# nv-dvl/nerfmatch

Measured on AMD Instinct MI355X. Metric: rays*samples/sec, higher is better.
Workload: dtype fp16x3 (fp16 MFMA on hi/lo-split fp32 operands, three products per fp32 product, fp32 accumulate; fp32 everywhere else)

## Files before the change

### nerfmatch_amd/csrc/nerf_fwd_bf16.hip

```cpp
#include "nerf_split_chain.h"

namespace {
using namespace nmbf;
using nmsample::HALF_PI_F32, nmsample::SCAN_TILE, nmsample::frustum, nmsample::ray_consts, nmsample::lift_var, nmsample::ipe_fast, nmsample::view_row_value;
using nmsample::alpha_of, nmsample::trans_factor, nmsample::sigmoid, nmsample::scan_before_barrier, nmsample::scan_after_barrier, nmsample::scan_carry;
using nmsample::first_max;
static_assert(TILE == SCAN_TILE, "the compositing scan of nerf_sample.h spans two wavefronts");

template <int PART>
__device__ __forceinline__ void tap_prefetch(Ctx& cx) {
  if constexpr (PART == 0) __builtin_amdgcn_s_barrier();
  const char* src = reinterpret_cast<const char*>(cx.tapw);
#pragma unroll
  for (int q = (PART == 0 ? 0 : 4); q < (PART == 0 ? 4 : 7); ++q) {
    const char* sp = src + q * 4096;
    const float* dp = q < 4 ? cx.tap_ring + q * 1024 : cx.tap_ipe + (q - 4) * 1024;
    const unsigned lds = (unsigned)__builtin_amdgcn_readfirstlane((int)(unsigned)(size_t)(const __attribute__((address_space(3))) float*)dp);
    unsigned m0_saved;
    asm volatile("s_mov_b32 %0, m0\n\ts_mov_b32 m0, %1\n\tglobal_load_lds_dwordx4 %2, off\n\tglobal_load_lds_dwordx4 %2, off offset:1024\n\t"
                 "global_load_lds_dwordx4 %2, off offset:2048\n\tglobal_load_lds_dwordx4 %2, off offset:3072\n\ts_mov_b32 m0, %0"
                 : "=&s"(m0_saved) : "s"(lds), "v"(sp) : "memory");
  }
}

// ... 67 lines not shown
#pragma unroll
    for (int i = 0; i < 8; ++i) s3[8 * b + i] = o[i];
  }
  float lo8[8], hi8[8];
#pragma unroll
  for (int i = 0; i < 8; ++i) { lo8[i] = s3[i]; hi8[i] = s3[8 + i]; }
  quad_add8<2>(lo8); quad_add8<2>(hi8);
  float s4[8];
#pragma unroll
  for (int i = 0; i < 8; ++i) s4[i] = (lane & 2) ? hi8[i] : lo8[i];
  float t8[8] = {s4[0], s4[1], s4[2], s4[3], s4[4], s4[5], s4[6], s4[7]};
  quad_add8<1>(t8);
  return (lane & 1) ? f32x4{t8[4], t8[5], t8[6], t8[7]} : f32x4{t8[0], t8[1], t8[2], t8[3]};
}
__device__ __forceinline__ f32x4 reduce_scatter_32rows(float (&v)[128], int lane) {
  float s1[64];
#pragma unroll
  for (int i = 0; i < 64; ++i) s1[i] = reduce_scatter_step16(v[i], v[64 + i]);
  return reduce_scatter_16pairs(s1, lane);
}

#define NM_MLP_DONE_WAIT() __builtin_amdgcn_s_waitcnt(0x0070)
#define NM_EPI_BARRIER() asm volatile("s_waitcnt lgkmcnt(0)\n\ts_barrier" ::: "memory")
template <int P>
__device__ __forceinline__ void nerf_fwd_body(const NerfArgs& a) {
  __shared__ __attribute__((aligned(16))) float sm[LDS_TOTAL];
  float* const sm_small = sm + LDS_SMALL;
  float* const ring = sm + LDS_RING;
  float* const sm_ipe = sm + LDS_IPE;
  float* const sm_sigma = sm + LDS_SCR;
  float* const sm_rgb = sm_sigma + TILE;
  float* const sm_t0 = sm_rgb + 3 * TILE;
  float* const sm_t1 = sm_t0 + TILE;
  float* const sm_mean = sm_t1 + TILE;
  float* const sm_dn = sm_mean + 3 * TILE;
  float* const sm_w = sm_dn + TILE;
  float* const sm_misc = sm_w + TILE;
  float* const sm_part = sm_misc + 32;
  float* const sm_feat = sm + LDS_FEAT;
  float* const sm_ex = sm + LDS_EX;
  int* const sm_lray = reinterpret_cast<int*>(sm + LDS_LEFT);
  float* const sm_lT = sm + LDS_LEFT + TILE;
  unsigned* const sm_rng = reinterpret_cast<unsigned*>(sm + LDS_RNG);

  const int tid = threadIdx.x, lane = tid & 63, wave = tid >> 6, s = lane & 31, hi = lane >> 5;
  const bool tail_ok = a.left && !(a.tail_viol && *a.tail_viol != 0);
  const int S = a.S, R = a.R;
  const int Sa = tail_ok ? a.Sa : S;
// ... 68 lines not shown
      sm_dn[js] = dnorm;
    }

    ring_open<P>(blob_slots, ring, wave, lane);

    {
      const float ipe_scale = sm_small[OFF_INSCALE];
      const float phl = hi ? HALF_PI_F32 : 0.f;
      park_ipe<P>(sm_ipe + wave * (XS * 2 * 64 * 4) + lane * 4, [&](int idx) {
        const int ax = idx % 3;
        const float sc = (float)(1 << (idx / 3));
        float v = ipe_fast(mean[ax] * sc + phl, var[ax], sc);
        if constexpr (P == 2) v *= ipe_scale;
        return v;
      });
    }

    TRACE(2);
    Ctx cx;
    cx.blob_slots = blob_slots; cx.ring = ring; cx.sm_small = sm_small;
    cx.tapw = reinterpret_cast<f32x4*>(a.ws) + ((size_t)blockIdx.x * 4 + wave) * 32 * 64 + lane;
    cx.nslots = nslots; cx.wave = wave; cx.lane = lane; cx.hi = hi; cx.tap = need_tap ? tap : -1; cx.g = 0; cx.sig_part = 0.f;
    cx.vmax = 0.f; cx.rng = sm_rng + tid; cx.sc = 1.f;
    const bool early = need_rgb && !lo_pass && tap == 7 && a.feat && !a.sfeat;
    cx.tap_pref = need_tap && !lo_pass && !early; cx.rgb = need_rgb;
    cx.tap_ring = ring + wave * SLOT_FLOATS; cx.tap_ipe = sm_ipe + wave * (XS * 2 * 64 * 4);
    if constexpr (is_split<P>()) {
      ring_open_wait<P>(cx);
    } else {
      ring_acquire<P>(blob_slots, 0, nslots, ring, wave, lane);
    }
    load_half<P>(cx.opA, ring, lane, 0);
    if constexpr (P == 1) load_half<1>(cx.opB, ring, lane, 1);
    const float* ipe_src = sm_ipe + wave * (XS * 2 * 64 * 4) + lane * 4;

    auto composite_weights = [&]() __attribute__((always_inline)) {
      const int tid2 = launder(threadIdx.x), lane2 = tid2 & 63, wave2 = tid2 >> 6;
      float alpha = 0.f, incl = 1.f;
      if (tid2 < TILE) {
        alpha = alpha_of(sm_sigma[tid2], (sm_t1[tid2] - sm_t0[tid2]) * sm_dn[tid2]);
        incl = scan_before_barrier(trans_factor(alpha), lane2, wave2, SP, sm_misc);
      }
      NM_EPI_BARRIER();
      if (tid2 < TILE) {
        const float excl = scan_after_barrier(incl, lane2, wave2, SP, sm_misc, carryT);
        sm_w[tid2] = alpha * excl;
        const int r2 = tid2 / SP, ray2 = bid * nr + r2;
// ... 62 lines not shown
#pragma unroll
      for (int cq = 0; cq < HS; ++cq) {
        const f32x4 b0 = *reinterpret_cast<const f32x4*>(bl + (cq >> 2) * 32 + 8 * (cq & 3));
        const f32x4 b1 = *reinterpret_cast<const f32x4*>(bl + (4 + (cq >> 2)) * 32 + 8 * (cq & 3));
#pragma unroll
        for (int e = 0; e < 4; ++e) {
          const float x = mult * __builtin_fmaxf(__builtin_fmaf(c.hv[4 * cq + e], s7, b0[e]), 0.f);
          const float y = mult * __builtin_fmaxf(__builtin_fmaf(c.hv[64 + 4 * cq + e], s7, b1[e]), 0.f);
          s1[4 * cq + e] = reduce_scatter_step16(x, y);
        }
      }
      const f32x4 sum4 = reduce_scatter_16pairs(s1, jl);
      const int r = jl & 31;
      float* prow = sm_feat + (jl >> 5) * 256 + 4 * hl;
      *reinterpret_cast<f32x4*>(prow + (r >> 2) * 32 + 16 * ((r >> 1) & 1) + 8 * (r & 1)) = sum4;
    };
    const Tap7InRegisters<decltype(tap7_early)> tap7{early, tap7_early};
    f32x16 acc[8];
    ipe_steps<P, true>(acc, cx, ipe_src);
    finish_layer<P>(acc, 0, cx);
    TRACE(3);
#pragma unroll 1
    for (int l = 1; l < 8; ++l) {
      layer_pass<P>(acc, l, cx, ipe_src, tap7);
      TRACE(3 + l);
    }
    float c_r = 0.f, c_g = 0.f, c_b = 0.f;
    if (!need_rgb) {
      if (cx.tap == 7) dump_tap(7, cx);
      NM_MLP_DONE_WAIT();
      if (cx.tap_pref) tap_prefetch<0>(cx);
      alpha_head(cx);
      if (cx.tap_pref) tap_prefetch<1>(cx);
    } else {
      const int hh = launder(lane) >> 5;
      const float* exr = sm_ex + launder(rl) * 48 + 8 * hh;
      f32x16 av[4];
      views_hidden<P>(av, cx);
      fold_range<P>(cx, 7);
      bf16x8 exh[VS], exl[VS];
#pragma unroll
      for (int e = 0; e < VS; ++e) {
        float v8[8];
        if (!lo_pass) {
          const f32x4 e0 = *reinterpret_cast<const f32x4*>(exr + 16 * e), e1 = *reinterpret_cast<const f32x4*>(exr + 16 * e + 4);
          v8[0] = e0[0]; v8[1] = e0[1]; v8[2] = e0[2]; v8[3] = e0[3]; v8[4] = e1[0]; v8[5] = e1[1]; v8[6] = e1[2]; v8[7] = e1[3];
        } else {
          const float* rq = a.rays + (size_t)launder(rc) * 12 + 8;
          const float vd0 = rq[0], vd1 = rq[1], vd2 = rq[2];
#pragma unroll
          for (int i = 0; i < 8; ++i) {
            const int f = 16 * e + 8 * hh + i;
            const int ax = f % 3;
            float v = view_row_value(f, ax == 0 ? vd0 : ax == 1 ? vd1 : vd2, a.app_row);
            if constexpr (P == 2) v *= sm_small[OFF_INSCALE + (f < 27 ? 1 : 2)];
            v8[i] = v;
          }
        }
        if constexpr (is_split<P>()) split8_p<P>(v8, exh[e], exl[e]);
        else exh[e] = exl[e] = pack8_f16(v8);
      }
// ... 188 lines not shown
      if (q == 0) { if (a.acc) a.acc[ray2] = red_acc; }
      else if (q <= 3) { if (a.rgb && need_rgb) a.rgb[(size_t)ray2 * 3 + (q - 1)] = a.white_bg ? red_acc + (1.0f - accv) : red_acc; }
      else if (q == 4) { if (a.depth) a.depth[ray2] = red_acc; }
      else { if (a.pts) a.pts[(size_t)ray2 * 3 + (q - 5)] = red_acc; }
    }
  }
  TRACE(17);
  if (left) nleft += (R - bid * nr) < nr ? (R - bid * nr) : nr;
  bid += gridDim.x;
  }
  if constexpr (P == 2) {
    __syncthreads();
    if (a.status && tid < NRANGE) {
      unsigned m = 0u;
      for (int i = 0; i < 256; ++i) m = max(m, sm_rng[tid * 256 + ((i + 32 * tid) & 255)]);
      if (m) atomicMax(reinterpret_cast<unsigned*>(a.status) + 1 + tid, m);
      if (m >= __float_as_uint(F16_MAX)) atomicOr(a.status, 1);
    }
  }
}

__global__ void __launch_bounds__(256, 1) nerf_fwd_bf16x3_kernel(NerfArgs a) { nerf_fwd_body<0>(a); }
__global__ void __launch_bounds__(256, 1) nerf_fwd_fp16x1_kernel(NerfArgs a) { nerf_fwd_body<1>(a); }
__global__ void __launch_bounds__(256, 1) nerf_fwd_fp16x3_kernel(NerfArgs a) { nerf_fwd_body<2>(a); }

}

extern "C" size_t nm_nerf_workspace_bytes_bf16x3(void) { return (size_t)WS_WORKGROUPS * TILE * 256 * sizeof(float); }

static int nerf_fwd_split(int mode, const void* blob, const float* rays, const float* t, const float* app_row, int R, int S, int tap_layer,
                          int white_bg, float var_scale, int flags, float* weights, float* feat, float* pts, float* rgb, float* depth,
                          float* acc, float* raw, float* sample_feat, void* workspace, const int* zero_tail_violation, nmStream_t stream,
                          int* status = nullptr) {
  NM_CHECK_ARG(blob && rays && t && weights && R > 0 && S > 0);
  if (!(S == 32 || S == 64 || (S % 128) == 0)) return NM_ERR_UNSUPPORTED;
  if (tap_layer > 7) return NM_ERR_ARG;
  if ((feat || sample_feat) && !workspace) return NM_ERR_WORKSPACE;
  NerfArgs a;
  a.ws = (float*)workspace;
  a.blob = (const char*)blob; a.rays = rays; a.t = t; a.app_row = app_row;
  a.weights = weights; a.feat = feat; a.pts = pts; a.rgb = rgb; a.depth = depth; a.acc = acc; a.raw = raw; a.sfeat = sample_feat;
  a.R = R; a.S = S; a.tap = tap_layer; a.white_bg = white_bg; a.flags = flags; a.var_scale = var_scale;
  a.status = status;
  const bool zero_tail = (flags & NM_NERF_ZERO_TAIL) && (S == 64 || S == 128 || (S >= 256 && S % 256 == 0)) && !raw && !sample_feat &&
                         !(flags & NM_NERF_FEAT_MAX);
  a.Sa = zero_tail ? S / 2 : S;
  a.left = zero_tail ? 1 : 0;
  const int SP = a.Sa < TILE ? a.Sa : TILE, nr = TILE / SP;
  a.ntiles = (R + nr - 1) / nr;
  const int SPf = S < TILE ? S : TILE, nrf = TILE / SPf;
  a.ntiles_full = (R + nrf - 1) / nrf;
  a.tail_viol = zero_tail ? zero_tail_violation : nullptr;
  const int ncu = nm_stream_cus(stream);
  const int grid = a.ntiles < ncu ? a.ntiles : (ncu < WS_WORKGROUPS ? ncu : WS_WORKGROUPS);
  if (mode == 1) nerf_fwd_fp16x1_kernel<<<grid, 256, 0, (hipStream_t)stream>>>(a);
  else if (mode == 2) nerf_fwd_fp16x3_kernel<<<grid, 256, 0, (hipStream_t)stream>>>(a);
  else nerf_fwd_bf16x3_kernel<<<grid, 256, 0, (hipStream_t)stream>>>(a);
  return nm_launch_status();
}

extern "C" int nm_nerf_fwd_bf16x3(const void* blob, const float* rays, const float* t, const float* app_row, int R, int S,
                                  int tap_layer, int white_bg, float var_scale, int flags, float* weights, float* feat, float* pts,
                                  float* rgb, float* depth, float* acc, float* raw, float* sample_feat, void* workspace,
                                  const int* zero_tail_violation, nmStream_t stream) {
  return nerf_fwd_split(0, blob, rays, t, app_row, R, S, tap_layer, white_bg, var_scale, flags, weights, feat, pts, rgb, depth, acc, raw,
                        sample_feat, workspace, zero_tail_violation, stream);
}

extern "C" int nm_nerf_fwd_fp16x1(const void* blob, const float* rays, const float* t, const float* app_row, int R, int S,
                                  int tap_layer, int white_bg, float var_scale, int flags, float* weights, float* feat, float* pts,
                                  float* rgb, float* depth, float* acc, float* raw, float* sample_feat, void* workspace,
                                  const int* zero_tail_violation, nmStream_t stream) {
  return nerf_fwd_split(1, blob, rays, t, app_row, R, S, tap_layer, white_bg, var_scale, flags, weights, feat, pts, rgb, depth, acc, raw,
                        sample_feat, workspace, zero_tail_violation, stream);
}

extern "C" int nm_nerf_fwd_fp16x3(const void* blob, const float* rays, const float* t, const float* app_row, int R, int S,
                                  int tap_layer, int white_bg, float var_scale, int flags, float* weights, float* feat, float* pts,
                                  float* rgb, float* depth, float* acc, float* raw, float* sample_feat, void* workspace,
// ... 5 lines not shown
```

### nerfmatch_amd/csrc/nerf_split_chain.h

```cpp
#pragma once
#include "nerf_bf16_common.h"

namespace nmbf {

template <int P> constexpr bool is_bf16() { return P == 0 || P == 4; }
template <int P> constexpr bool has_gates() { return P == 4; }
typedef _Float16 f16x8 __attribute__((ext_vector_type(8)));
typedef _Float16 f16x2 __attribute__((ext_vector_type(2)));
template <int P>
__device__ __forceinline__ f32x16 mfma_p(const bf16x8& a, const bf16x8& b, const f32x16& c) {
  if constexpr (is_bf16<P>()) return MFMA_BF16(a, b, c);
  else return __builtin_amdgcn_mfma_f32_32x32x16_f16(__builtin_bit_cast(f16x8, a), __builtin_bit_cast(f16x8, b), c, 0, 0, 0);
}
template <int P> constexpr bool is_split() { return P != 1; }
template <int P> constexpr int slot_bytes() { return is_split<P>() ? SLOT_BYTES : SLOT_BYTES / 2; }
template <int P> constexpr int slot_floats() { return slot_bytes<P>() / 4; }
template <int P> constexpr int ring_slots() { return is_split<P>() ? NRING : 2 * NRING; }
template <int P> constexpr int ring_ahead() { return is_split<P>() ? 4 : 6; }
constexpr float F16_MAX = 65504.0f;
__device__ __forceinline__ void split8_f16(const float (&v)[8], bf16x8& hi, bf16x8& lo) {
  f16x8 h8, l8;
#pragma unroll
  for (int i = 0; i < 8; ++i) {
    const float c = __builtin_amdgcn_fmed3f(v[i], -F16_MAX, F16_MAX);
// ... 49 lines not shown
  auto* dst = (__attribute__((address_space(3))) void*)(ring_slot<P>(ring, g) + wave * (slot_floats<P>() / 4));
  __builtin_amdgcn_global_load_lds(src, dst, 16, 0, 0);
  __builtin_amdgcn_global_load_lds(src, dst, 16, 1024, 0);
  if constexpr (is_split<P>()) {
    __builtin_amdgcn_global_load_lds(src, dst, 16, 2048, 0);
    __builtin_amdgcn_global_load_lds(src, dst, 16, 3072, 0);
  }
}

template <int P>
__device__ __forceinline__ void ring_acquire(const char* blob_slots, int g, int nslots, float* ring, int wave, int lane) {
  if constexpr (is_split<P>()) {
    NM_WAIT_VMCNT(4);
  } else {
    NM_WAIT_VMCNT(10);
  }
  __builtin_amdgcn_s_barrier();
  if constexpr (is_split<P>()) dma_slot<P>(blob_slots, g + ring_ahead<P>(), ring, wave, lane);
}

__device__ __forceinline__ void ring_acquire_two() {
  asm volatile("s_waitcnt vmcnt(0) lgkmcnt(0)" ::: "memory");
  __builtin_amdgcn_s_barrier();
}

__device__ __forceinline__ void ring_acquire_pair(const char* blob_slots, int g, float* ring, int wave, int lane) {
  NM_WAIT_VMCNT(6);
  __builtin_amdgcn_s_barrier();
  dma_slot<1>(blob_slots, g + 6, ring, wave, lane);
  dma_slot<1>(blob_slots, g + 7, ring, wave, lane);
}

struct OpHalf {
  bf16x8 h[4], l[4];
};

template <int P>
__device__ __forceinline__ void load_half(OpHalf& d, const float* slot, int lane, int p) {
  const u32x4* s4 = reinterpret_cast<const u32x4*>(slot) + lane;
#pragma unroll
  for (int o = 0; o < 4; ++o) {
    if constexpr (is_split<P>()) {
      d.h[o] = __builtin_bit_cast(bf16x8, s4[((4 * p + o) * 2 + 0) * 64]);
      d.l[o] = __builtin_bit_cast(bf16x8, s4[((4 * p + o) * 2 + 1) * 64]);
    } else {
      d.h[o] = __builtin_bit_cast(bf16x8, s4[(4 * p + o) * 64]);
    }
  }
}

struct Ctx {
  const char* blob_slots;
  float* ring;
  const float* sm_small;
  f32x4* tapw;
  bool tap_pref;
  bool rgb;
  float* tap_ring;
  float* tap_ipe;
  int nslots, wave, lane, hi;
  int tap;
  int g;
  unsigned dma_voff;
  unsigned dma_lds;
  OpHalf opA;
  OpHalf opB;
  f32x4 hb0, hb1;
  Unit xn;
  float sig_part;
  float sc;
  float vmax;
  unsigned* rng;
  u32x4* gptr;
  unsigned gbits[4];
  float hv[128];
};

template <int P>
__device__ __forceinline__ void ring_request(const Ctx& cx, int g, int j) {
  const int slot = g + 2 + (j >> 2);
  const char* base = cx.blob_slots + (size_t)slot * slot_bytes<P>();
  const unsigned lds = cx.dma_lds + (unsigned)(slot & (ring_slots<P>() - 1)) * slot_bytes<P>();
  unsigned m0_saved;
#define NM_DMA_PIECE(OFS)                                                                                                        \
  asm volatile("s_mov_b32 %0, m0\n\ts_mov_b32 m0, %1\n\tglobal_load_lds_dwordx4 %2, %3 offset:" #OFS "\n\ts_mov_b32 m0, %0" \
               : "=&s"(m0_saved) : "s"(lds), "v"(cx.dma_voff), "s"(base) : "memory")
  switch (j & 3) {
    case 0: NM_DMA_PIECE(0); break;
    case 1: NM_DMA_PIECE(1024); break;
    case 2: NM_DMA_PIECE(2048); break;
    default: NM_DMA_PIECE(3072); break;
  }
#undef NM_DMA_PIECE
}
template <int P>
__device__ __forceinline__ void ring_open(const char* blob_slots, float* ring, int wave, int lane) {
#pragma unroll
  for (int g0 = 0; g0 < (is_split<P>() ? 2 : ring_ahead<P>()); ++g0) dma_slot<P>(blob_slots, g0, ring, wave, lane);
}
template <int P>
__device__ __forceinline__ void ring_open_wait(Ctx& cx) {
  cx.dma_voff = (unsigned)(cx.wave * (slot_bytes<P>() / 4) + cx.lane * 16);
  const float* q = cx.ring + cx.wave * (slot_floats<P>() / 4);
  cx.dma_lds = (unsigned)__builtin_amdgcn_readfirstlane((int)(unsigned)(size_t)(const __attribute__((address_space(3))) float*)q);
  NM_WAIT_VMCNT(0);
  __builtin_amdgcn_s_barrier();
}

__device__ __forceinline__ unsigned gate_byte(const u32x4& h) {
  const unsigned w0 = h[0], w1 = h[1], w2 = h[2], w3 = h[3];
  unsigned m0, m1, m2, m3;
  const unsigned one = 0x00010001u;
  asm("v_pk_min_u16 %0, %1, %2" : "=v"(m0) : "v"(w0), "v"(one));
  asm("v_pk_min_u16 %0, %1, %2" : "=v"(m1) : "v"(w1), "v"(one));
  asm("v_pk_min_u16 %0, %1, %2" : "=v"(m2) : "v"(w2), "v"(one));
  asm("v_pk_min_u16 %0, %1, %2" : "=v"(m3) : "v"(w3), "v"(one));
  const unsigned t = m0 | (m1 << 1) | (m2 << 2) | (m3 << 3);
  return (t & 0xfu) | ((t >> 12) & 0xf0u);
}

template <bool BF, class W> __device__ __forceinline__ void unit_seq(W& w, int c);
template <bool EVEN, bool BF, class W> __device__ __forceinline__ void unit_step8(W& w, int t);
template <int P>
struct UnitWork {
  Ctx& cx;
  Unit& out;
  int u, lo_;
  float floor_v;
  f32x4 b0, b1;
  float sc;
  float v8[8];
  float f0, f1;
  float r0[4], r1[4];
  __device__ __forceinline__ void bias() {
    const int ob = u >> 1, m = u & 1;
    const float* bl = cx.sm_small + OFF_BIAS + lo_ * 256 + ob * 32 + 16 * m + 4 * cx.hi;
    b0 = *reinterpret_cast<const f32x4*>(bl); b1 = *reinterpret_cast<const f32x4*>(bl + 8);
  }
  __device__ __forceinline__ float act(int e, float b) const {
    const float h = cx.hv[(u >> 1) * 16 + 8 * (u & 1) + e];
    if constexpr (is_bf16<P>()) return __builtin_fmaxf(h + b, floor_v);
    else if constexpr (P == 1) return __builtin_amdgcn_fmed3f(h + b, floor_v, F16_MAX);
    else return __builtin_amdgcn_fmed3f(__builtin_fmaf(h, sc, b), floor_v, F16_MAX);
  }
  __device__ __forceinline__ void range(int j) {
    if constexpr (P == 2) asm("v_max3_f32 %0, |%1|, |%2|, %0" : "+v"(cx.vmax) : "v"(v8[j]), "v"(v8[4 + j]));
  }
  __device__ __forceinline__ void ra(int j) { v8[j] = act(j, b0[j]); pin(v8[j]); }
  __device__ __forceinline__ void rb(int j) { v8[4 + j] = act(4 + j, b1[j]); range(j); pin(v8[4 + j]); }
  __device__ __forceinline__ void relu(int j) {
    v8[j] = act(j, b0[j]); v8[4 + j] = act(4 + j, b1[j]);
    range(j);
    pin(v8[j]); pin(v8[4 + j]);
  }
  __device__ __forceinline__ void hi(int p) {
    unsigned hp;
    if constexpr (is_bf16<P>()) {
      hp = pack_bf16(v8[2 * p], v8[2 * p + 1]);
      f0 = __uint_as_float(hp << 16);
      f1 = __uint_as_float(hp & 0xffff0000u);
// ... 4 lines not shown
    if constexpr (is_bf16<P>()) { pin(f0); pin(f1); }
    out.h[p] = hp;
  }
  __device__ __forceinline__ void rem(int p) {
    if constexpr (is_bf16<P>()) {
      r0[p] = v8[2 * p] - f0; r1[p] = v8[2 * p + 1] - f1;
      pin(r0[p]); pin(r1[p]);
    } else {
      asm volatile("v_fma_mix_f32 %0, %1, -1.0, %2 op_sel:[0,0,0] op_sel_hi:[1,0,0]" : "=v"(r0[p]) : "v"(out.h[p]), "v"(v8[2 * p]));
      asm volatile("v_fma_mix_f32 %0, %1, -1.0, %2 op_sel:[1,0,0] op_sel_hi:[1,0,0]" : "=v"(r1[p]) : "v"(out.h[p]), "v"(v8[2 * p + 1]));
    }
  }
  __device__ __forceinline__ void lo(int p) {
    unsigned lp = is_bf16<P>() ? pack_bf16(r0[p], r1[p]) : pack_f16(r0[p], r1[p]);
    pin(lp);
    out.l[p] = lp;
  }
  __device__ __forceinline__ void gates() {
    if constexpr (has_gates<P>()) {
      const unsigned t = gate_byte(out.h);
      cx.gbits[u >> 2] |= t << (8 * (u & 3));
    }
  }
  __device__ __forceinline__ void seq(int c) { unit_seq<is_bf16<P>()>(*this, c); }
  template <bool EVEN> __device__ __forceinline__ void step8(int t) { unit_step8<EVEN, is_bf16<P>()>(*this, t); }
  __device__ __forceinline__ void prefetch() { bias(); }
  __device__ __forceinline__ void operator()(int j) {
    if (j < 4) relu(j);
    else if constexpr (P == 1) {
      if (j < 8) {
        unsigned hp = pack_f16(v8[2 * (j - 4)], v8[2 * (j - 4) + 1]);
        pin(hp);
        out.h[j - 4] = hp;
      }
    } else if (!(j & 1)) hi((j - 4) >> 1);
    else {
      rem((j - 5) >> 1); lo((j - 5) >> 1);
      if (j == 11) gates();
    }
  }
};
template <bool BF, class W>
__device__ __forceinline__ void unit_seq(W& w, int c) {
  switch (c) {
    case 0: w.bias(); break;
    case 2: w.ra(0); break;
    case 3: w.rb(0); break;
    case 4: w.ra(1); break;
// ... 25 lines not shown
      case 18: if constexpr (BF) { w.rem(2); } break;
      case 19: if constexpr (BF) { w.hi(3); w.lo(2); } break;
      case 20: if constexpr (BF) { w.rem(3); } break;
      case 21: if constexpr (BF) { w.lo(3); } break;
      case 22: if constexpr (BF) { w.gates(); } break;
      default: break;
    }
  }
}
template <int P>
__device__ __forceinline__ void fold_range(Ctx& cx, int slot) {
  if constexpr (P == 2) {
    const unsigned addr = (unsigned)(size_t)(const __attribute__((address_space(3))) unsigned*)(cx.rng + slot * 256);
    asm volatile("ds_max_u32 %0, %1" :: "v"(addr), "v"(__float_as_uint(cx.vmax)) : "memory");
    cx.vmax = 0.f;
  }
}
struct NoWork {
  __device__ __forceinline__ void prefetch() {}
  __device__ __forceinline__ void operator()(int) {}
  __device__ __forceinline__ void seq(int) {}
  template <bool EVEN> __device__ __forceinline__ void step8(int) {}
};
constexpr int take_n(int s) { return s == 0 ? 4 : s == 1 ? 2 : s <= 4 ? 3 : s == 10 ? 2 : 5; }
constexpr int take_before(int s) {
  int n = 0;
  for (int k = 0; k < s; ++k) n += take_n(k);
  return n;
}
constexpr int TAKE_HIDDEN = take_before(12);
__device__ __forceinline__ const float* unit0_bias(const Ctx& cx, int l) { return cx.sm_small + OFF_BIAS + l * 256 + 4 * cx.hi; }
template <int P>
struct AccTake {
  const f32x16 (&acc)[8];
  Ctx& cx;
  int l;
  __device__ __forceinline__ void prefetch() {}
  __device__ __forceinline__ void operator()(int j) {
#pragma unroll
    for (int k = 0; k < 8; ++k) {
      const int i = 8 * j + k;
      if (i < 64) cx.hv[i] = acc_read(acc[i >> 4][i & 15]);
    }
  }
  __device__ __forceinline__ void seq(int) {}
  template <bool EVEN> __device__ __forceinline__ void step8(int t) {
    if (t < 12) return;
    const int s = t - 12;
#pragma unroll
    for (int k = 0; k < take_n(s); ++k) {
      const int i = take_before(s) + k;
      cx.hv[i] = acc_read(acc[i >> 4][i & 15]);
    }
    if (s == 10) {
      const float* bl = unit0_bias(cx, l);
      cx.hb0 = *reinterpret_cast<const f32x4*>(bl); cx.hb1 = *reinterpret_cast<const f32x4*>(bl + 8);
    }
  }
};
template <int P>
__device__ __forceinline__ UnitWork<P> unit_work(int u, int lo, Ctx& cx, Unit& out) {
  return UnitWork<P>{cx, out, u, lo, lo < 8 ? 0.f : (!is_bf16<P>() ? -F16_MAX : -__builtin_inff()), {}, {}, cx.sc, {}, 0.f, 0.f, {}, {}};
}

template <int P>
__device__ __forceinline__ void finish_layer(const f32x16 (&acc)[8], int l, Ctx& cx) {
  if constexpr (is_split<P>()) {
#pragma unroll
    for (int i = TAKE_HIDDEN; i < 64; ++i) cx.hv[i] = acc_read(acc[i >> 4][i & 15]);
  }
#pragma unroll
  for (int ob = 4; ob < 8; ++ob)
#pragma unroll
    for (int r = 0; r < 16; ++r) cx.hv[ob * 16 + r] = acc_read(acc[ob][r]);
  if constexpr (P == 2)
    cx.sc = __builtin_bit_cast(float, __builtin_amdgcn_readfirstlane(__builtin_bit_cast(int, cx.sm_small[OFF_SCALE + l])));
  UnitWork<P> w = unit_work<P>(0, l, cx, cx.xn);
  if constexpr (is_split<P>()) {
    w.b0 = cx.hb0; w.b1 = cx.hb1;
#pragma unroll
    for (int j = 0; j < 4; ++j) w.relu(j);
#pragma unroll
    for (int p = 0; p < 4; ++p) {
      w.hi(p);
      if constexpr (is_bf16<P>()) w.rem(p);
    }
    if constexpr (!is_bf16<P>()) {
#pragma unroll
      for (int p = 0; p < 4; ++p) w.rem(p);
    }
#pragma unroll
    for (int p = 0; p < 4; ++p) w.lo(p);
    w.gates();
  } else {
    w.prefetch();
#pragma unroll
    for (int j = 0; j < 12; ++j) w(j);
  }
}

__device__ __forceinline__ void alpha_head(Ctx& cx) {
  const float* bl = cx.sm_small + OFF_BIAS + 7 * 256 + 4 * cx.hi;
  const float* wa = cx.sm_small + OFF_WALPHA + 4 * cx.hi;
  const float s7 = cx.sm_small[OFF_SCALE + 7];
  float p0 = 0.f, p1 = 0.f, p2 = 0.f, p3 = 0.f;
#pragma unroll
  for (int ob = 0; ob < 8; ++ob)
#pragma unroll
    for (int q = 0; q < 4; ++q) {
      const f32x4 b = *reinterpret_cast<const f32x4*>(bl + ob * 32 + 8 * q);
      const f32x4 w4v = *reinterpret_cast<const f32x4*>(wa + ob * 32 + 8 * q);
      p0 = NM_FMA(__builtin_fmaxf(__builtin_fmaf(cx.hv[ob * 16 + 4 * q + 0], s7, b[0]), 0.f), w4v[0], p0);
      p1 = NM_FMA(__builtin_fmaxf(__builtin_fmaf(cx.hv[ob * 16 + 4 * q + 1], s7, b[1]), 0.f), w4v[1], p1);
      p2 = NM_FMA(__builtin_fmaxf(__builtin_fmaf(cx.hv[ob * 16 + 4 * q + 2], s7, b[2]), 0.f), w4v[2], p2);
      p3 = NM_FMA(__builtin_fmaxf(__builtin_fmaf(cx.hv[ob * 16 + 4 * q + 3], s7, b[3]), 0.f), w4v[3], p3);
    }
  cx.sig_part = (p0 + p1) + (p2 + p3);
}

__device__ __forceinline__ void dump_tap(int lo, Ctx& cx) {
  const float* bl = cx.sm_small + OFF_BIAS + lo * 256 + 4 * cx.hi;
  const float sl = cx.sm_small[OFF_SCALE + lo];
  auto* tp = (__attribute__((address_space(1))) f32x4*)cx.tapw;
#pragma unroll
  for (int ob = 0; ob < 8; ++ob) {
    f32x4 v[4];
#pragma unroll
    for (int q = 0; q < 4; ++q) {
      const f32x4 b = *reinterpret_cast<const f32x4*>(bl + ob * 32 + 8 * q);
#pragma unroll
      for (int e = 0; e < 4; ++e) v[q][e] = __builtin_fmaxf(__builtin_fmaf(cx.hv[ob * 16 + 4 * q + e], sl, b[e]), 0.f);
    }
#pragma unroll
    for (int q = 0; q < 4; ++q) tp[q * 64] = v[q];
    tp += 256;
    pin(tp);
  }
}

__device__ __forceinline__ bf16x8 load_op1(const float* slot, int lane, int blk) {
  return __builtin_bit_cast(bf16x8, (reinterpret_cast<const u32x4*>(slot) + lane)[blk * 64]);
// ... 19 lines not shown
  acc[5] = mfma_p<1>(B.h[1], x, FIRST ? zero : acc[5]); NM_SB;
  work(0); work(1); NM_SB;
  acc[6] = mfma_p<1>(B.h[2], x, FIRST ? zero : acc[6]); NM_SB;
  work(2); work(3); work(4); NM_SB;
  acc[7] = mfma_p<1>(B.h[3], x, FIRST ? zero : acc[7]); NM_SB;
  work(5); work(6); work(7); NM_SB;
  cx.g = g + 1;
}

template <int P>
__device__ __forceinline__ void load_pair(OpHalf& d, const float* slot, int lane, int p, int o) {
  const u32x4* s4 = reinterpret_cast<const u32x4*>(slot) + lane;
  d.h[o] = __builtin_bit_cast(bf16x8, s4[((4 * p + o) * 2 + 0) * 64]);
  d.l[o] = __builtin_bit_cast(bf16x8, s4[((4 * p + o) * 2 + 1) * 64]);
}
template <int P, bool FIRST>
__device__ __forceinline__ f32x16 mfma_k(int k, const OpHalf& a, const bf16x8& xh, const bf16x8& xl, const f32x16& c) {
  const f32x16 zero = {0.f, 0.f, 0.f, 0.f, 0.f, 0.f, 0.f, 0.f, 0.f, 0.f, 0.f, 0.f, 0.f, 0.f, 0.f, 0.f};
  if (k < 4) return mfma_p<P>(a.h[k], xh, FIRST ? zero : c);
  if (k < 8) return mfma_p<P>(a.h[k & 3], xl, c);
  return mfma_p<P>(a.l[k & 3], xh, c);
}

template <int P, bool FIRST, bool EVEN, class Work>
__device__ __forceinline__ void slot_step8(f32x16 (&acc)[8], Ctx& cx, const bf16x8& xh, const bf16x8& xl, Work work) {
  if constexpr (P == 1) {
    slot_step8_one<FIRST, EVEN>(acc, cx, xh, work);
    return;
  }
  const int g = cx.g;
  const OpHalf A = cx.opA;
  OpHalf B;
  const float* cur = cx.ring + (g & (NRING - 1)) * SLOT_FLOATS;
  const float* nxt = cx.ring + ((g + 1) & (NRING - 1)) * SLOT_FLOATS;
#pragma unroll
  for (int k = 0; k < 12; ++k) {
    acc[k & 3] = mfma_k<P, FIRST>(k, A, xh, xl, acc[k & 3]);
    __builtin_amdgcn_sched_barrier(0);
    if (k < 4) load_pair<P>(B, cur, cx.lane, 1, k);
    if constexpr (EVEN) {
      if (k >= 4) ring_request<P>(cx, g, k - 4);
    }
    work.template step8<EVEN>(k);
    __builtin_amdgcn_sched_barrier(0);
  }
  if constexpr (!EVEN) {
    ring_acquire_two();
    __builtin_amdgcn_sched_barrier(0);
  }
#pragma unroll
  for (int k = 0; k < 12; ++k) {
    acc[4 + (k & 3)] = mfma_k<P, FIRST>(k, B, xh, xl, acc[4 + (k & 3)]);
    __builtin_amdgcn_sched_barrier(0);
    if (k >= 1 && k <= 4) load_pair<P>(cx.opA, nxt, cx.lane, 0, k - 1);
    work.template step8<EVEN>(12 + k);
    __builtin_amdgcn_sched_barrier(0);
  }
  cx.g = g + 1;
}

template <bool FIRST, bool ACQ, class Work>
__device__ __forceinline__ void slot_step4_one(f32x16 (&acc)[4], Ctx& cx, const bf16x8& x, Work work) {
  const f32x16 zero = {0.f, 0.f, 0.f, 0.f, 0.f, 0.f, 0.f, 0.f, 0.f, 0.f, 0.f, 0.f, 0.f, 0.f, 0.f, 0.f};
  const int g = cx.g;
  const OpHalf C = cx.opA;
  const float* nxt = ring_slot<1>(cx.ring, g + 1);
  acc[0] = mfma_p<1>(C.h[0], x, FIRST ? zero : acc[0]); NM_SB;
  if constexpr (ACQ) ring_acquire_pair(cx.blob_slots, g, cx.ring, cx.wave, cx.lane);
  NM_SB;
  acc[1] = mfma_p<1>(C.h[1], x, FIRST ? zero : acc[1]); NM_SB;
#pragma unroll
  for (int o = 0; o < 4; ++o) cx.opA.h[o] = load_op1(nxt, cx.lane, o);
  work.prefetch(); NM_SB;
  acc[2] = mfma_p<1>(C.h[2], x, FIRST ? zero : acc[2]); NM_SB;
  work(0); work(1); work(2); work(3); NM_SB;
  acc[3] = mfma_p<1>(C.h[3], x, FIRST ? zero : acc[3]); NM_SB;
  work(4); work(5); work(6); work(7); NM_SB;
// ... 19 lines not shown
      if (k >= 4) ring_request<P>(cx, g, k - 4);
    }
    work.seq(k);
    __builtin_amdgcn_sched_barrier(0);
  }
  cx.g = g + 1;
}

template <int P, bool FIRST, bool EVEN, class W0, class W1>
__device__ __forceinline__ void slot_step4x2(f32x16 (&av)[4], Ctx& cx, const bf16x8& x0h, const bf16x8& x0l, Unit& u1, W0 w0, W1 w1) {
  const int g = cx.g;
  const OpHalf A = cx.opA;
  OpHalf B;
  const float* cur = cx.ring + (g & (NRING - 1)) * SLOT_FLOATS;
  const float* nxt = cx.ring + ((g + 1) & (NRING - 1)) * SLOT_FLOATS;
#pragma unroll
  for (int k = 0; k < 12; ++k) {
    av[k & 3] = mfma_k<P, FIRST>(k, A, x0h, x0l, av[k & 3]);
    __builtin_amdgcn_sched_barrier(0);
    if (k >= 1 && k <= 4) load_pair<P>(B, cur, cx.lane, 1, k - 1);
    if constexpr (EVEN) {
      if (k >= 4) ring_request<P>(cx, g, k - 4);
    }
    w0.seq(k);
    __builtin_amdgcn_sched_barrier(0);
  }
  if constexpr (!EVEN) {
    ring_acquire_two();
    __builtin_amdgcn_sched_barrier(0);
  }
  const bf16x8 x1h = __builtin_bit_cast(bf16x8, u1.h), x1l = __builtin_bit_cast(bf16x8, u1.l);
#pragma unroll
  for (int k = 0; k < 12; ++k) {
    av[k & 3] = mfma_k<P, false>(k, B, x1h, x1l, av[k & 3]);
    __builtin_amdgcn_sched_barrier(0);
    if (k >= 1 && k <= 4) load_pair<P>(cx.opA, nxt, cx.lane, 0, k - 1);
    w1.seq(k);
    __builtin_amdgcn_sched_barrier(0);
  }
  cx.g = g + 1;
}

template <int P>
__device__ __forceinline__ void views_hidden(f32x16 (&av)[4], Ctx& cx) {
  if constexpr (is_split<P>()) {
#pragma unroll
    for (int sl = 0; sl < HS / 2; ++sl) {
      const Unit x0 = cx.xn;
      Unit u1;
      const bf16x8 x0h = __builtin_bit_cast(bf16x8, x0.h), x0l = __builtin_bit_cast(bf16x8, x0.l);
      if (sl == 0) slot_step4x2<P, true, true>(av, cx, x0h, x0l, u1, unit_work<P>(1, 7, cx, u1), unit_work<P>(2, 7, cx, cx.xn));
      else if (sl + 1 == HS / 2) slot_step4x2<P, false, false>(av, cx, x0h, x0l, u1, unit_work<P>(2 * sl + 1, 7, cx, u1), NoWork{});
      else if (sl & 1) slot_step4x2<P, false, false>(av, cx, x0h, x0l, u1, unit_work<P>(2 * sl + 1, 7, cx, u1), unit_work<P>(2 * sl + 2, 7, cx, cx.xn));
      else slot_step4x2<P, false, true>(av, cx, x0h, x0l, u1, unit_work<P>(2 * sl + 1, 7, cx, u1), unit_work<P>(2 * sl + 2, 7, cx, cx.xn));
    }
  } else {
#pragma unroll
    for (int ks = 0; ks < HS; ks += 2) {
      {
        const Unit xc = cx.xn;
        if (ks == 0) slot_step4<P, true, true>(av, cx, __builtin_bit_cast(bf16x8, xc.h), __builtin_bit_cast(bf16x8, xc.l), unit_work<P>(ks + 1, 7, cx, cx.xn));
        else slot_step4<P, false, true>(av, cx, __builtin_bit_cast(bf16x8, xc.h), __builtin_bit_cast(bf16x8, xc.l), unit_work<P>(ks + 1, 7, cx, cx.xn));
      }
      {
        const Unit xc = cx.xn;
        if (ks + 2 < HS) slot_step4<P, false, false>(av, cx, __builtin_bit_cast(bf16x8, xc.h), __builtin_bit_cast(bf16x8, xc.l), unit_work<P>(ks + 2, 7, cx, cx.xn));
        else slot_step4<P, false, false>(av, cx, __builtin_bit_cast(bf16x8, xc.h), __builtin_bit_cast(bf16x8, xc.l), NoWork{});
      }
    }
  }
}
template <int P>
__device__ __forceinline__ void views_extras(f32x16 (&av)[4], Ctx& cx, const bf16x8 (&eh)[VS], const bf16x8 (&el)[VS], bool no_app) {
  if constexpr (is_split<P>()) {
    Unit u1;
    u1.h = __builtin_bit_cast(u32x4, eh[1]); u1.l = __builtin_bit_cast(u32x4, el[1]);
    slot_step4x2<P, false, true>(av, cx, eh[0], el[0], u1, NoWork{}, NoWork{});
    if (!no_app) slot_step4<P, false, false>(av, cx, eh[2], el[2], NoWork{});
  } else {
    slot_step4<P, false, true>(av, cx, eh[0], el[0], NoWork{});
    slot_step4<P, false, false>(av, cx, eh[1], el[1], NoWork{});
    if (!no_app) slot_step4<P, false, true>(av, cx, eh[2], el[2], NoWork{});
  }
}

template <int P, bool FIRST>
__device__ __forceinline__ void ipe_steps(f32x16 (&acc)[8], Ctx& cx, const float* ipe_src, int l = FIRST ? 0 : 5) {
  auto operand = [&](int m, bf16x8& ph, bf16x8& pl) {
    ph = __builtin_bit_cast(bf16x8, *reinterpret_cast<const u32x4*>(ipe_src + (is_split<P>() ? (m * 2 + 0) : m) * 256));
    pl = ph;
    if constexpr (is_split<P>()) pl = __builtin_bit_cast(bf16x8, *reinterpret_cast<const u32x4*>(ipe_src + (m * 2 + 1) * 256));
  };
#pragma unroll
  for (int m = 0; m < XS; m += 2) {
    bf16x8 ph, pl;
    operand(m, ph, pl);
    if (m == 0) slot_step8<P, FIRST, true>(acc, cx, ph, pl, NoWork{});
    else slot_step8<P, false, true>(acc, cx, ph, pl, NoWork{});
    operand(m + 1, ph, pl);
    if (m + 2 == XS) slot_step8<P, false, false>(acc, cx, ph, pl, AccTake<P>{acc, cx, l});
    else slot_step8<P, false, false>(acc, cx, ph, pl, NoWork{});
  }
}

struct Tap7Workspace {
  static constexpr bool on = false;
  __device__ __forceinline__ void fn(Ctx&) const {}
};
template <class F>
struct Tap7InRegisters {
  bool on;
  F fn;
};

template <int P, class Tap7 = Tap7Workspace>
__device__ __forceinline__ void layer_pass(f32x16 (&acc)[8], int l, Ctx& cx, const float* ipe_src, const Tap7& tap7 = Tap7()) {
  if (l - 1 == cx.tap) dump_tap(l - 1, cx);
#pragma unroll
  for (int ks = 0; ks < HS; ks += 2) {
    {
      const Unit xc = cx.xn;
      if (ks == 0) slot_step8<P, true, true>(acc, cx, __builtin_bit_cast(bf16x8, xc.h), __builtin_bit_cast(bf16x8, xc.l), unit_work<P>(ks + 1, l - 1, cx, cx.xn));
      else slot_step8<P, false, true>(acc, cx, __builtin_bit_cast(bf16x8, xc.h), __builtin_bit_cast(bf16x8, xc.l), unit_work<P>(ks + 1, l - 1, cx, cx.xn));
    }
    {
      const Unit xc = cx.xn;
      if (ks + 2 < HS) slot_step8<P, false, false>(acc, cx, __builtin_bit_cast(bf16x8, xc.h), __builtin_bit_cast(bf16x8, xc.l), unit_work<P>(ks + 2, l - 1, cx, cx.xn));
      else slot_step8<P, false, false>(acc, cx, __builtin_bit_cast(bf16x8, xc.h), __builtin_bit_cast(bf16x8, xc.l), AccTake<P>{acc, cx, l});
    }
  }
  fold_range<P>(cx, l - 1);
  if constexpr (has_gates<P>()) {
    cx.gptr[(l - 1) * 256] = u32x4{cx.gbits[0], cx.gbits[1], cx.gbits[2], cx.gbits[3]};
    cx.gbits[0] = cx.gbits[1] = cx.gbits[2] = cx.gbits[3] = 0u;
  }
  if (l == 5) ipe_steps<P, false>(acc, cx, ipe_src);
  finish_layer<P>(acc, l, cx);
  if (l == 7) {
    if (cx.rgb) {
      if (cx.tap == 7 && !tap7.on) dump_tap(7, cx);
      alpha_head(cx);
      if (tap7.on) tap7.fn(cx);
    }
  }
}

}
```

Before: 385.8 million.

## Overlap fp16x3 density head, bias and ring requests with MFMA K-loops

```diff
diff --git a/nerfmatch_amd/csrc/nerf_fwd_bf16.hip b/nerfmatch_amd/csrc/nerf_fwd_bf16.hip
--- a/nerfmatch_amd/csrc/nerf_fwd_bf16.hip
+++ b/nerfmatch_amd/csrc/nerf_fwd_bf16.hip
@@ -113,8 +113,9 @@
 
 #define NM_MLP_DONE_WAIT() __builtin_amdgcn_s_waitcnt(0x0070)
 #define NM_EPI_BARRIER() asm volatile("s_waitcnt lgkmcnt(0)\n\ts_barrier" ::: "memory")
-template <int P>
+template <int P, bool TAP7 = true>
 __device__ __forceinline__ void nerf_fwd_body(const NerfArgs& a) {
+  constexpr bool DENS = P == 2 && !TAP7;
   __shared__ __attribute__((aligned(16))) float sm[LDS_TOTAL];
   float* const sm_small = sm + LDS_SMALL;
   float* const ring = sm + LDS_RING;
@@ -229,7 +230,7 @@
     cx.tapw = reinterpret_cast<f32x4*>(a.ws) + ((size_t)blockIdx.x * 4 + wave) * 32 * 64 + lane;
     cx.nslots = nslots; cx.wave = wave; cx.lane = lane; cx.hi = hi; cx.tap = need_tap ? tap : -1; cx.g = 0; cx.sig_part = 0.f;
     cx.vmax = 0.f; cx.rng = sm_rng + tid; cx.sc = 1.f;
-    const bool early = need_rgb && !lo_pass && tap == 7 && a.feat && !a.sfeat;
+    const bool early = TAP7 && need_rgb && !lo_pass && tap == 7 && a.feat && !a.sfeat;
     cx.tap_pref = need_tap && !lo_pass && !early; cx.rgb = need_rgb;
     cx.tap_ring = ring + wave * SLOT_FLOATS; cx.tap_ipe = sm_ipe + wave * (XS * 2 * 64 * 4);
     if constexpr (is_split<P>()) {
@@ -338,7 +339,7 @@
     TRACE(3);
 #pragma unroll 1
     for (int l = 1; l < 8; ++l) {
-      layer_pass<P>(acc, l, cx, ipe_src, tap7);
+      layer_pass<P, DENS>(acc, l, cx, ipe_src, tap7);
       TRACE(3 + l);
     }
     float c_r = 0.f, c_g = 0.f, c_b = 0.f;
@@ -352,7 +353,10 @@
       const int hh = launder(lane) >> 5;
       const float* exr = sm_ex + launder(rl) * 48 + 8 * hh;
       f32x16 av[4];
-      views_hidden<P>(av, cx);
+      if constexpr (DENS) {
+        views_hidden<P, true>(av, cx);
+        dens_close(cx);
+      } else views_hidden<P>(av, cx);
       fold_range<P>(cx, 7);
       bf16x8 exh[VS], exl[VS];
 #pragma unroll
@@ -587,7 +591,8 @@
 
 __global__ void __launch_bounds__(256, 1) nerf_fwd_bf16x3_kernel(NerfArgs a) { nerf_fwd_body<0>(a); }
 __global__ void __launch_bounds__(256, 1) nerf_fwd_fp16x1_kernel(NerfArgs a) { nerf_fwd_body<1>(a); }
-__global__ void __launch_bounds__(256, 1) nerf_fwd_fp16x3_kernel(NerfArgs a) { nerf_fwd_body<2>(a); }
+__global__ void __launch_bounds__(256, 1) nerf_fwd_fp16x3_kernel(NerfArgs a) { nerf_fwd_body<2, false>(a); }
+__global__ void __launch_bounds__(256, 1) nerf_fwd_fp16x3_tap7_kernel(NerfArgs a) { nerf_fwd_body<2, true>(a); }
 
 }
 
@@ -619,7 +624,11 @@
   const int ncu = nm_stream_cus(stream);
   const int grid = a.ntiles < ncu ? a.ntiles : (ncu < WS_WORKGROUPS ? ncu : WS_WORKGROUPS);
   if (mode == 1) nerf_fwd_fp16x1_kernel<<<grid, 256, 0, (hipStream_t)stream>>>(a);
-  else if (mode == 2) nerf_fwd_fp16x3_kernel<<<grid, 256, 0, (hipStream_t)stream>>>(a);
+  else if (mode == 2) {
+    const bool tap7_early = !(flags & NM_NERF_SKIP_RGB) && (tap_layer < 0 || tap_layer == 7) && feat && !sample_feat;
+    if (tap7_early) nerf_fwd_fp16x3_tap7_kernel<<<grid, 256, 0, (hipStream_t)stream>>>(a);
+    else nerf_fwd_fp16x3_kernel<<<grid, 256, 0, (hipStream_t)stream>>>(a);
+  }
   else nerf_fwd_bf16x3_kernel<<<grid, 256, 0, (hipStream_t)stream>>>(a);
   return nm_launch_status();
 }
diff --git a/nerfmatch_amd/csrc/nerf_split_chain.h b/nerfmatch_amd/csrc/nerf_split_chain.h
--- a/nerfmatch_amd/csrc/nerf_split_chain.h
+++ b/nerfmatch_amd/csrc/nerf_split_chain.h
@@ -95,6 +95,11 @@
 __device__ __forceinline__ void ring_acquire_two() {
   asm volatile("s_waitcnt vmcnt(0) lgkmcnt(0)" ::: "memory");
   __builtin_amdgcn_s_barrier();
+}
+
+template <int P>
+__device__ __forceinline__ void lds_retire() {
+  if constexpr (P == 2) __builtin_amdgcn_s_waitcnt(0xC07F);
 }
 
 __device__ __forceinline__ void ring_acquire_pair(const char* blob_slots, int g, float* ring, int wave, int lane) {
@@ -141,6 +146,9 @@
   f32x4 hb0, hb1;
   Unit xn;
   float sig_part;
+  float dp[4];
+  float dv[3], dw[3];
+  f32x4 nb0, nb1;
   float sc;
   float vmax;
   unsigned* rng;
@@ -166,6 +174,7 @@
   }
 #undef NM_DMA_PIECE
 }
+template <int P> constexpr bool request_early() { return P == 2; }
 template <int P>
 __device__ __forceinline__ void ring_open(const char* blob_slots, float* ring, int wave, int lane) {
 #pragma unroll
@@ -194,7 +203,7 @@
 
 template <bool BF, class W> __device__ __forceinline__ void unit_seq(W& w, int c);
 template <bool EVEN, bool BF, class W> __device__ __forceinline__ void unit_step8(W& w, int t);
-template <int P>
+template <int P, bool DENS = false>
 struct UnitWork {
   Ctx& cx;
   Unit& out;
@@ -205,10 +214,45 @@
   float v8[8];
   float f0, f1;
   float r0[4], r1[4];
+  f32x4 wa0, wa1;
+  __device__ __forceinline__ static void dens_fma(float& p, float v, float w) { asm volatile("v_fma_f32 %0, %1, %2, %0" : "+v"(p) : "v"(v), "v"(w)); }
+  __device__ __forceinline__ void dens_seq(int c) {
+    if constexpr (DENS) {
+      switch (c) {
+        case 0: {
+          const float* wl = cx.sm_small + OFF_WALPHA + (u >> 1) * 32 + 16 * (u & 1) + 4 * cx.hi;
+          wa0 = *reinterpret_cast<const f32x4*>(wl); wa1 = *reinterpret_cast<const f32x4*>(wl + 8);
+        } break;
+        case 1:
+          dens_fma(cx.dp[1], cx.dv[0], cx.dw[0]); dens_fma(cx.dp[2], cx.dv[1], cx.dw[1]); dens_fma(cx.dp[3], cx.dv[2], cx.dw[2]);
+          break;
+        case 7: dens_fma(cx.dp[0], v8[0], wa0[0]); break;
+        case 10: dens_fma(cx.dp[0], v8[4], wa1[0]); break;
+        case 11:
+          dens_fma(cx.dp[1], v8[1], wa0[1]); dens_fma(cx.dp[2], v8[2], wa0[2]); dens_fma(cx.dp[3], v8[3], wa0[3]);
+          cx.dv[0] = v8[5]; cx.dw[0] = wa1[1]; cx.dv[1] = v8[6]; cx.dw[1] = wa1[2]; cx.dv[2] = v8[7]; cx.dw[2] = wa1[3];
+          break;
+        default: break;
+      }
+    }
+  }
   __device__ __forceinline__ void bias() {
+    if constexpr (P == 2) {
+      b0 = cx.nb0; b1 = cx.nb1;
+      return;
+    }
     const int ob = u >> 1, m = u & 1;
     const float* bl = cx.sm_small + OFF_BIAS + lo_ * 256 + ob * 32 + 16 * m + 4 * cx.hi;
     b0 = *reinterpret_cast<const f32x4*>(bl); b1 = *reinterpret_cast<const f32x4*>(bl + 8);
+  }
+  __device__ __forceinline__ void bias_next() {
+    if constexpr (P == 2) {
+      if (u + 1 < HS) {
+        const int ob = (u + 1) >> 1, m = (u + 1) & 1;
+        const float* bl = cx.sm_small + OFF_BIAS + lo_ * 256 + ob * 32 + 16 * m + 4 * cx.hi;
+        cx.nb0 = *reinterpret_cast<const f32x4*>(bl); cx.nb1 = *reinterpret_cast<const f32x4*>(bl + 8);
+      }
+    }
   }
   __device__ __forceinline__ float act(int e, float b) const {
     const float h = cx.hv[(u >> 1) * 16 + 8 * (u & 1) + e];
@@ -259,8 +303,14 @@
       cx.gbits[u >> 2] |= t << (8 * (u & 3));
     }
   }
-  __device__ __forceinline__ void seq(int c) { unit_seq<is_bf16<P>()>(*this, c); }
-  template <bool EVEN> __device__ __forceinline__ void step8(int t) { unit_step8<EVEN, is_bf16<P>()>(*this, t); }
+  __device__ __forceinline__ void seq(int c) {
+    unit_seq<is_bf16<P>()>(*this, c); dens_seq(c);
+    if (c == 11) bias_next();
+  }
+  template <bool EVEN> __device__ __forceinline__ void step8(int t) {
+    unit_step8<EVEN, is_bf16<P>()>(*this, t);
+    if (t == 23) bias_next();
+  }
   __device__ __forceinline__ void prefetch() { bias(); }
   __device__ __forceinline__ void operator()(int j) {
     if (j < 4) relu(j);
@@ -332,6 +382,18 @@
   __device__ __forceinline__ void seq(int) {}
   template <bool EVEN> __device__ __forceinline__ void step8(int) {}
 };
+template <int T>
+struct IpeFetch {
+  const float* src;
+  int m;
+  bf16x8& ph;
+  bf16x8& pl;
+  template <bool EVEN> __device__ __forceinline__ void step8(int t) {
+    if (t != T) return;
+    ph = __builtin_bit_cast(bf16x8, *reinterpret_cast<const u32x4*>(src + (m * 2 + 0) * 256));
+    pl = __builtin_bit_cast(bf16x8, *reinterpret_cast<const u32x4*>(src + (m * 2 + 1) * 256));
+  }
+};
 constexpr int take_n(int s) { return s == 0 ? 4 : s == 1 ? 2 : s <= 4 ? 3 : s == 10 ? 2 : 5; }
 constexpr int take_before(int s) {
   int n = 0;
@@ -368,9 +430,9 @@
     }
   }
 };
-template <int P>
-__device__ __forceinline__ UnitWork<P> unit_work(int u, int lo, Ctx& cx, Unit& out) {
-  return UnitWork<P>{cx, out, u, lo, lo < 8 ? 0.f : (!is_bf16<P>() ? -F16_MAX : -__builtin_inff()), {}, {}, cx.sc, {}, 0.f, 0.f, {}, {}};
+template <int P, bool DENS = false>
+__device__ __forceinline__ UnitWork<P, DENS> unit_work(int u, int lo, Ctx& cx, Unit& out) {
+  return UnitWork<P, DENS>{cx, out, u, lo, lo < 8 ? 0.f : (!is_bf16<P>() ? -F16_MAX : -__builtin_inff()), {}, {}, cx.sc, {}, 0.f, 0.f, {}, {}, {}, {}};
 }
 
 template <int P>
@@ -386,6 +448,10 @@
   if constexpr (P == 2)
     cx.sc = __builtin_bit_cast(float, __builtin_amdgcn_readfirstlane(__builtin_bit_cast(int, cx.sm_small[OFF_SCALE + l])));
   UnitWork<P> w = unit_work<P>(0, l, cx, cx.xn);
+  if constexpr (P == 2) {
+    const float* bl = unit0_bias(cx, l) + 16;
+    cx.nb0 = *reinterpret_cast<const f32x4*>(bl); cx.nb1 = *reinterpret_cast<const f32x4*>(bl + 8);
+  }
   if constexpr (is_split<P>()) {
     w.b0 = cx.hb0; w.b1 = cx.hb1;
 #pragma unroll
@@ -427,6 +493,34 @@
     }
   cx.sig_part = (p0 + p1) + (p2 + p3);
 }
+
+__device__ __forceinline__ void dens_open(Ctx& cx) {
+  const float* bl = cx.sm_small + OFF_BIAS + 7 * 256 + 4 * cx.hi;
+  const float* wa = cx.sm_small + OFF_WALPHA + 4 * cx.hi;
+  const f32x4 b0 = *reinterpret_cast<const f32x4*>(bl), b1 = *reinterpret_cast<const f32x4*>(bl + 8);
+  const f32x4 w0 = *reinterpret_cast<const f32x4*>(wa), w1 = *reinterpret_cast<const f32x4*>(wa + 8);
+  float v[8];
+#pragma unroll
+  for (int j = 0; j < 4; ++j) {
+    v[j] = __builtin_fmaxf(__builtin_fmaf(cx.hv[j], cx.sc, b0[j]), 0.f);
+    v[4 + j] = __builtin_fmaxf(__builtin_fmaf(cx.hv[4 + j], cx.sc, b1[j]), 0.f);
+  }
+#pragma unroll
+  for (int j = 0; j < 4; ++j) cx.dp[j] = NM_FMA(v[j], w0[j], 0.f);
+  cx.dp[0] = NM_FMA(v[4], w1[0], cx.dp[0]);
+#pragma unroll
+  for (int j = 0; j < 3; ++j) { cx.dv[j] = v[5 + j]; cx.dw[j] = w1[1 + j]; }
+}
+struct DensTail {
+  Ctx& cx;
+  __device__ __forceinline__ void seq(int c) {
+    if (c == 1) {
+#pragma unroll
+      for (int j = 0; j < 3; ++j) UnitWork<2, true>::dens_fma(cx.dp[1 + j], cx.dv[j], cx.dw[j]);
+    }
+  }
+};
+__device__ __forceinline__ void dens_close(Ctx& cx) { cx.sig_part = (cx.dp[0] + cx.dp[1]) + (cx.dp[2] + cx.dp[3]); }
 
 __device__ __forceinline__ void dump_tap(int lo, Ctx& cx) {
   const float* bl = cx.sm_small + OFF_BIAS + lo * 256 + 4 * cx.hi;
@@ -492,7 +586,7 @@
   return mfma_p<P>(a.l[k & 3], xh, c);
 }
 
-template <int P, bool FIRST, bool EVEN, class Work>
+template <int P, bool FIRST, bool EVEN, bool RQE = false, class Work>
 __device__ __forceinline__ void slot_step8(f32x16 (&acc)[8], Ctx& cx, const bf16x8& xh, const bf16x8& xl, Work work) {
   if constexpr (P == 1) {
     slot_step8_one<FIRST, EVEN>(acc, cx, xh, work);
@@ -508,8 +602,11 @@
     acc[k & 3] = mfma_k<P, FIRST>(k, A, xh, xl, acc[k & 3]);
     __builtin_amdgcn_sched_barrier(0);
     if (k < 4) load_pair<P>(B, cur, cx.lane, 1, k);
-    if constexpr (EVEN) {
+    if constexpr (EVEN && !RQE) {
       if (k >= 4) ring_request<P>(cx, g, k - 4);
+    }
+    if constexpr (EVEN && RQE) {
+      if (k == 4 || k == 5) ring_request<P>(cx, g, k + 2);
     }
     work.template step8<EVEN>(k);
     __builtin_amdgcn_sched_barrier(0);
@@ -523,6 +620,10 @@
     acc[4 + (k & 3)] = mfma_k<P, FIRST>(k, B, xh, xl, acc[4 + (k & 3)]);
     __builtin_amdgcn_sched_barrier(0);
     if (k >= 1 && k <= 4) load_pair<P>(cx.opA, nxt, cx.lane, 0, k - 1);
+    if constexpr (!EVEN && RQE) {
+      if (k >= 5 && k <= 10) ring_request<P>(cx, g + 1, k - 5);
+    }
+    if (k == 11) lds_retire<P>();
     work.template step8<EVEN>(12 + k);
     __builtin_amdgcn_sched_barrier(0);
   }
@@ -588,6 +689,7 @@
     if constexpr (EVEN) {
       if (k >= 4) ring_request<P>(cx, g, k - 4);
     }
+    if (k == 11) lds_retire<P>();
     w0.seq(k);
     __builtin_amdgcn_sched_barrier(0);
   }
@@ -601,24 +703,28 @@
     av[k & 3] = mfma_k<P, false>(k, B, x1h, x1l, av[k & 3]);
     __builtin_amdgcn_sched_barrier(0);
     if (k >= 1 && k <= 4) load_pair<P>(cx.opA, nxt, cx.lane, 0, k - 1);
+    if (k == 11) lds_retire<P>();
     w1.seq(k);
     __builtin_amdgcn_sched_barrier(0);
   }
   cx.g = g + 1;
 }
 
-template <int P>
+template <int P, bool DENS = false>
 __device__ __forceinline__ void views_hidden(f32x16 (&av)[4], Ctx& cx) {
+  static_assert(!DENS || P == 2, "the density head accumulates in the views K-loop in fp16x3 only");
   if constexpr (is_split<P>()) {
 #pragma unroll
     for (int sl = 0; sl < HS / 2; ++sl) {
       const Unit x0 = cx.xn;
       Unit u1;
       const bf16x8 x0h = __builtin_bit_cast(bf16x8, x0.h), x0l = __builtin_bit_cast(bf16x8, x0.l);
-      if (sl == 0) slot_step4x2<P, true, true>(av, cx, x0h, x0l, u1, unit_work<P>(1, 7, cx, u1), unit_work<P>(2, 7, cx, cx.xn));
-      else if (sl + 1 == HS / 2) slot_step4x2<P, false, false>(av, cx, x0h, x0l, u1, unit_work<P>(2 * sl + 1, 7, cx, u1), NoWork{});
-      else if (sl & 1) slot_step4x2<P, false, false>(av, cx, x0h, x0l, u1, unit_work<P>(2 * sl + 1, 7, cx, u1), unit_work<P>(2 * sl + 2, 7, cx, cx.xn));
-      else slot_step4x2<P, false, true>(av, cx, x0h, x0l, u1, unit_work<P>(2 * sl + 1, 7, cx, u1), unit_work<P>(2 * sl + 2, 7, cx, cx.xn));
+      if (sl == 0) slot_step4x2<P, true, true>(av, cx, x0h, x0l, u1, unit_work<P, DENS>(1, 7, cx, u1), unit_work<P, DENS>(2, 7, cx, cx.xn));
+      else if (sl + 1 == HS / 2) {
+        if constexpr (DENS) slot_step4x2<P, false, false>(av, cx, x0h, x0l, u1, unit_work<P, DENS>(2 * sl + 1, 7, cx, u1), DensTail{cx});
+        else slot_step4x2<P, false, false>(av, cx, x0h, x0l, u1, unit_work<P>(2 * sl + 1, 7, cx, u1), NoWork{});
+      } else if (sl & 1) slot_step4x2<P, false, false>(av, cx, x0h, x0l, u1, unit_work<P, DENS>(2 * sl + 1, 7, cx, u1), unit_work<P, DENS>(2 * sl + 2, 7, cx, cx.xn));
+      else slot_step4x2<P, false, true>(av, cx, x0h, x0l, u1, unit_work<P, DENS>(2 * sl + 1, 7, cx, u1), unit_work<P, DENS>(2 * sl + 2, 7, cx, cx.xn));
     }
   } else {
 #pragma unroll
@@ -657,6 +763,18 @@
     pl = ph;
     if constexpr (is_split<P>()) pl = __builtin_bit_cast(bf16x8, *reinterpret_cast<const u32x4*>(ipe_src + (m * 2 + 1) * 256));
   };
+  if constexpr (P == 2) {
+    bf16x8 ph, pl, qh, ql;
+    operand(0, ph, pl);
+#pragma unroll
+    for (int m = 0; m < XS; m += 2) {
+      if (m == 0) slot_step8<P, FIRST, true>(acc, cx, ph, pl, IpeFetch<17>{ipe_src, m + 1, qh, ql});
+      else slot_step8<P, false, true, true>(acc, cx, ph, pl, IpeFetch<6>{ipe_src, m + 1, qh, ql});
+      if (m + 2 == XS) slot_step8<P, false, false>(acc, cx, qh, ql, AccTake<P>{acc, cx, l});
+      else slot_step8<P, false, false, true>(acc, cx, qh, ql, IpeFetch<4>{ipe_src, m + 2, ph, pl});
+    }
+    return;
+  }
 #pragma unroll
   for (int m = 0; m < XS; m += 2) {
     bf16x8 ph, pl;
@@ -679,7 +797,7 @@
   F fn;
 };
 
-template <int P, class Tap7 = Tap7Workspace>
+template <int P, bool DENS = false, class Tap7 = Tap7Workspace>
 __device__ __forceinline__ void layer_pass(f32x16 (&acc)[8], int l, Ctx& cx, const float* ipe_src, const Tap7& tap7 = Tap7()) {
   if (l - 1 == cx.tap) dump_tap(l - 1, cx);
 #pragma unroll
@@ -687,11 +805,11 @@
     {
       const Unit xc = cx.xn;
       if (ks == 0) slot_step8<P, true, true>(acc, cx, __builtin_bit_cast(bf16x8, xc.h), __builtin_bit_cast(bf16x8, xc.l), unit_work<P>(ks + 1, l - 1, cx, cx.xn));
-      else slot_step8<P, false, true>(acc, cx, __builtin_bit_cast(bf16x8, xc.h), __builtin_bit_cast(bf16x8, xc.l), unit_work<P>(ks + 1, l - 1, cx, cx.xn));
+      else slot_step8<P, false, true, request_early<P>()>(acc, cx, __builtin_bit_cast(bf16x8, xc.h), __builtin_bit_cast(bf16x8, xc.l), unit_work<P>(ks + 1, l - 1, cx, cx.xn));
     }
     {
       const Unit xc = cx.xn;
-      if (ks + 2 < HS) slot_step8<P, false, false>(acc, cx, __builtin_bit_cast(bf16x8, xc.h), __builtin_bit_cast(bf16x8, xc.l), unit_work<P>(ks + 2, l - 1, cx, cx.xn));
+      if (ks + 2 < HS) slot_step8<P, false, false, request_early<P>()>(acc, cx, __builtin_bit_cast(bf16x8, xc.h), __builtin_bit_cast(bf16x8, xc.l), unit_work<P>(ks + 2, l - 1, cx, cx.xn));
       else slot_step8<P, false, false>(acc, cx, __builtin_bit_cast(bf16x8, xc.h), __builtin_bit_cast(bf16x8, xc.l), AccTake<P>{acc, cx, l});
     }
   }
@@ -705,7 +823,8 @@
   if (l == 7) {
     if (cx.rgb) {
       if (cx.tap == 7 && !tap7.on) dump_tap(7, cx);
-      alpha_head(cx);
+      if constexpr (DENS) dens_open(cx);
+      else alpha_head(cx);
       if (tap7.on) tap7.fn(cx);
     }
   }
```

After: 400.1 million, median of 6. +3.7%, better.
